# AaltoML/vi-diffusion-processes

Measured on AMD Instinct MI355X. Metric: ELBO steps/sec (T=100k, d=6) at 1/2/4/8 GPU; HBM GB/s vs roofline, higher is better.
Workload: dtype f64; 1 GPU; CVI-DP site-update loop (CVISitesSDE: update_data_sites + update_girsanov_sites + classic_elbo) on double-well SDE trajectories, T=100000, d=6, 64 trajectories per GPU, observation every 50 steps, correlated observation noise (full d x d data sites); trajectories_per_gpu=64, T=100000, d=6, total_trajectories=64

## Files before the change

include/mfgm.h:

```cpp
#ifndef MFGM_H
#define MFGM_H

#include <stddef.h>
#include <stdint.h>

#ifdef __cplusplus
extern "C" {
#endif

typedef struct mfgm_plan mfgm_plan;

#define MFGM_VEC 0
#define MFGM_FULL 1
#define MFGM_SYM 2
#define MFGM_TRI 3

int mfgm_plan_create(int B, int T, int d, int R0, int Rup, mfgm_plan** out);
void mfgm_plan_destroy(mfgm_plan* plan);
int mfgm_plan_describe(const mfgm_plan* plan, int* out6);
size_t mfgm_plan_workspace_bytes(const mfgm_plan* plan);
size_t mfgm_packed_doubles(const mfgm_plan* plan, int kind);

int mfgm_pack(const mfgm_plan* plan, int kind, const double* natural, int n_nodes, double* packed, void* stream);
int mfgm_unpack(const mfgm_plan* plan, int kind, const double* packed, double* natural, int n_nodes, void* stream);
// ... 112 lines not shown
                        double* quad, double* L2, double* y2, void* ws, int* info, void* stream);
int mfgm_cq_factor_pair_stage(const mfgm_plan* plan, int stage, const mfgm_cq_state* q, const mfgm_cq_state* q_next, double* L, double* y,
                              double* L2, double* y2, void* ws, int* info, void* stream);
size_t mfgm_cq_heads_scratch_doubles(const mfgm_plan* plan, int stride);
int mfgm_cq_factor_pair_heads(const mfgm_plan* plan, int stride, const mfgm_cq_state* q, const mfgm_cq_state* q_next, double* L, double* y,
                              double* logdet, double* quad, double* L2, double* y2, double* scratch, size_t scratch_doubles, void* ws, int* info,
                              void* stream);
int mfgm_cq_factor_pair_heads_stage(const mfgm_plan* plan, int stage, int stride, const mfgm_cq_state* q, const mfgm_cq_state* q_next,
                                    double* L, double* y, double* L2, double* y2, double* scratch, size_t scratch_doubles, void* ws, int* info,
                                    void* stream);
int mfgm_cq_selinv_girsanov_alt(const mfgm_plan* plan, int only_level, const mfgm_cq_state* q, const double* L2, const double* y2,
                                const mfgm_sde_params* prm, double* dyn_out, void* ws, void* stream);
int mfgm_cq_selinv_kl(const mfgm_plan* plan, int only_level, const mfgm_cq_state* q, const double* L, const double* y,
                      const mfgm_sde_params* prm, double* Sig, double* x, double* kl_part, double* obs_mu, double* obs_cov, void* ws,
                      void* stream);
int mfgm_mvn_ve_compact(int B, int n_per, int d, const double* mu, const double* cov, const double* y, const double* Sinv, double cst,
                        double* ve, void* stream);

#define MFGM_QUAD_NTHETA 40
typedef struct mfgm_quad_drift {
    int kind, d, nh, pad_;
    double theta[MFGM_QUAD_NTHETA];
    double dt;
    double W[6];
    double logdetQp;
    double mu0[3];
    double P0inv[6];
    double logdetP0;
    double clip_lo, clip_hi;
} mfgm_quad_drift;
// ... 360 lines not shown
```

vi-diffusion-processes_amd/_lib.py:

```python
import ctypes
import os

_HERE = os.path.dirname(os.path.abspath(__file__))
LIB_PATH = os.environ.get("MFGM_LIB") or os.path.join(_HERE, "csrc", "libmfgm.so")

VEC, FULL, SYM, TRI = 0, 1, 2, 3
FACTOR_MATERN12, FACTOR_MATERN32, FACTOR_MATERN52, FACTOR_CONSTANT, FACTOR_HARMONIC = 1, 2, 3, 4, 5
LIK_BERNOULLI, LIK_POISSON, LIK_GAUSSIAN = 1, 2, 3

_lib = None

EXPORTS = {
    "mfgm_version": (ctypes.c_char_p, []),
    "mfgm_plan_create": (ctypes.c_int, [ctypes.c_int] * 5 + [ctypes.POINTER(ctypes.c_void_p)]),
    "mfgm_plan_destroy": (None, [ctypes.c_void_p]),
    "mfgm_plan_describe": (ctypes.c_int, [ctypes.c_void_p, ctypes.POINTER(ctypes.c_int)]),
    "mfgm_plan_workspace_bytes": (ctypes.c_size_t, [ctypes.c_void_p]),
    "mfgm_packed_doubles": (ctypes.c_size_t, [ctypes.c_void_p, ctypes.c_int]),
    "mfgm_pack": (ctypes.c_int, [ctypes.c_void_p, ctypes.c_int, ctypes.c_void_p, ctypes.c_int, ctypes.c_void_p,
                                 ctypes.c_void_p]),
    "mfgm_unpack": (ctypes.c_int, [ctypes.c_void_p, ctypes.c_int, ctypes.c_void_p, ctypes.c_void_p, ctypes.c_int,
                                   ctypes.c_void_p]),
    "mfgm_packed_factor": (ctypes.c_int, [ctypes.c_void_p] * 4 + [ctypes.c_double] * 3 + [ctypes.c_void_p] * 8),
    "mfgm_packed_selinv": (ctypes.c_int, [ctypes.c_void_p] * 9),
# ... 70 lines not shown
    "mfgm_cq_slots": (ctypes.c_int, [ctypes.c_void_p, ctypes.c_void_p, ctypes.c_int, ctypes.c_void_p, ctypes.c_void_p, ctypes.c_void_p]),
    "mfgm_cq_factor": (ctypes.c_int, [ctypes.c_void_p] * 9),
    "mfgm_cq_factor_pipelined": (ctypes.c_int, [ctypes.c_void_p] * 8 + [ctypes.c_int] + [ctypes.c_void_p] * 3),
    "mfgm_quad_linearize": (ctypes.c_int, [ctypes.c_void_p, ctypes.c_int] + [ctypes.c_void_p] * 6),
    "mfgm_quad_kl_scratch_doubles": (ctypes.c_size_t, [ctypes.c_int] * 4),
    "mfgm_quad_kl": (ctypes.c_int, [ctypes.c_void_p, ctypes.c_int, ctypes.c_int] + [ctypes.c_void_p] * 11),
    "mfgm_quad_vdp_lagrange": (ctypes.c_int, [ctypes.c_int] * 3 + [ctypes.c_double] * 2 + [ctypes.c_void_p] * 8),
    "mfgm_quad_esde": (ctypes.c_int, [ctypes.c_void_p, ctypes.c_int] + [ctypes.c_void_p] * 12),
    "mfgm_cq_factor_stage": (ctypes.c_int, [ctypes.c_void_p, ctypes.c_int] + [ctypes.c_void_p] * 6),
    "mfgm_cq_selinv_girsanov": (ctypes.c_int, [ctypes.c_void_p, ctypes.c_int] + [ctypes.c_void_p] * 7),
    "mfgm_cq_factor_pair": (ctypes.c_int, [ctypes.c_void_p] * 12),
    "mfgm_cq_factor_pair_stage": (ctypes.c_int, [ctypes.c_void_p, ctypes.c_int] + [ctypes.c_void_p] * 9),
    "mfgm_cq_heads_scratch_doubles": (ctypes.c_size_t, [ctypes.c_void_p, ctypes.c_int]),
    "mfgm_cq_factor_pair_heads": (ctypes.c_int, [ctypes.c_void_p, ctypes.c_int] + [ctypes.c_void_p] * 9 + [ctypes.c_size_t] + [ctypes.c_void_p] * 3),
    "mfgm_cq_factor_pair_heads_stage": (ctypes.c_int, [ctypes.c_void_p, ctypes.c_int, ctypes.c_int] + [ctypes.c_void_p] * 7 + [ctypes.c_size_t] + [ctypes.c_void_p] * 3),
    "mfgm_cq_selinv_girsanov_alt": (ctypes.c_int, [ctypes.c_void_p, ctypes.c_int] + [ctypes.c_void_p] * 7),
    "mfgm_cq_selinv_kl": (ctypes.c_int, [ctypes.c_void_p, ctypes.c_int] + [ctypes.c_void_p] * 11),
    "mfgm_mvn_ve_compact": (ctypes.c_int, [ctypes.c_int] * 3 + [ctypes.c_void_p] * 4 + [ctypes.c_double, ctypes.c_void_p, ctypes.c_void_p]),
    "mfgm_kf_sites_loglik": (ctypes.c_int, [ctypes.c_void_p] * 15),
    "mfgm_kf_sites_predict": (ctypes.c_int, [ctypes.c_void_p] * 16),
    "mfgm_kf_sites_elbo": (ctypes.c_int, [ctypes.c_void_p] * 9 + [ctypes.c_double] + [ctypes.c_void_p] * 6),
    "mfgm_kf_sites_predict_factored": (ctypes.c_int, [ctypes.c_void_p] * 11),
    "mfgm_sparse_theta": (ctypes.c_int, [ctypes.c_int, ctypes.c_int] + [ctypes.c_void_p] * 9),
    "mfgm_sparse_predict": (ctypes.c_int, [ctypes.c_void_p] * 7),
    "mfgm_cond_predict": (ctypes.c_int, [ctypes.c_int] * 3 + [ctypes.c_void_p] * 11),
    "mfgm_sparse_site_update": (ctypes.c_int, [ctypes.c_void_p] * 3 + [ctypes.c_double] + [ctypes.c_void_p] * 3),
    "mfgm_packed_naturals_to_ssm": (ctypes.c_int, [ctypes.c_void_p] * 11),
    "mfgm_bidiag_scratch_doubles": (ctypes.c_size_t, [ctypes.c_int] * 3),
    "mfgm_bidiag_solve": (ctypes.c_int, [ctypes.c_int] * 3 + [ctypes.c_void_p] * 4 + [ctypes.c_int, ctypes.c_void_p, ctypes.c_void_p]),
    "mfgm_btd_matvec": (ctypes.c_int, [ctypes.c_int] * 3 + [ctypes.c_void_p] * 4 + [ctypes.c_int, ctypes.c_int, ctypes.c_void_p]),
# ... 186 lines not shown
```

vi-diffusion-processes_amd/csrc/mfgm_api_sweeps.hip:

```cpp
#include "mfgm_internal.h"
#include "mfgm_sweeps.h"
#include "mfgm_rows.h"
#include "mfgm_girsanov.h"
#include "mfgm_cq.h"
#include "mfgm_kf.h"

using namespace mfgm;

namespace {

template <int D>
int launch_reduce(const SweepArgs& a, bool has_rhs, bool has_corr, hipStream_t st) {
    dim3 grid(a.lv.Lpad / 64), block(64);
    if (has_rhs) {
        if (has_corr) hipLaunchKernelGGL((k_reduce<D, true, true>), grid, block, 0, st, a);
        else hipLaunchKernelGGL((k_reduce<D, true, false>), grid, block, 0, st, a);
    } else {
        if (has_corr) hipLaunchKernelGGL((k_reduce<D, false, true>), grid, block, 0, st, a);
        else hipLaunchKernelGGL((k_reduce<D, false, false>), grid, block, 0, st, a);
    }
    MFGM_CHECK_LAUNCH();
    return 0;
}

// ... 319 lines not shown
            if (a0.lv.nt >= 2) hipLaunchKernelGGL((k_forward_cq<D, 2>), grid, block, 0, st, a0, q);
            else hipLaunchKernelGGL((k_forward_cq<D>), grid, block, 0, st, a0, q);
        }
        MFGM_CHECK_LAUNCH();
        if (next && !side && !rides) {
            hipLaunchKernelGGL((k_reduce_cq_lean<D>), grid, block, 0, st, an, *next);
            MFGM_CHECK_LAUNCH();
        }
    }
    if (logdet || quad) return sum_level0_partials(P, ws, P.lv[0].Lpad, logdet, quad, st);
    return 0;
}

template <int D>
int cq_factor_pair_impl(const Plan& P, const CqArgs& q, const CqArgs& q2, double* Lg, double* yg, double* logdet, double* quad, double* L2,
                        double* y2, double* ws, int* info, hipStream_t st, int only_stage = -1, double* park = nullptr, int stride = 0) {
    const auto on = [&](int s) { return only_stage < 0 || only_stage == s; };
    const size_t sh = P.off_pair - P.off_Dhat[1];
    double* ws2 = ws + sh;
    SweepArgs a0;
    memset(&a0, 0, sizeof(a0));
    a0.lv = P.lv[0];
    a0.info = info;
    a0.aD = -2.0; a0.aS = -1.0; a0.aR = 1.0;
    a0.Lg = Lg; a0.yg = yg;
    a0.part = (logdet || quad) ? ws + P.off_part[0] : nullptr;
    SweepArgs a1 = a0;
    a1.Lg = L2; a1.yg = y2; a1.part = nullptr;
    bind_up(P, 0, ws, a0);
    bind_up(P, 0, ws2, a1);
    dim3 grid(a0.lv.Lpad / 64), block(64);
    if (on(0) && park) {
        hipLaunchKernelGGL((k_reduce_cq_interior<D>), grid, block, 0, st, a0, q, park, stride);
        MFGM_CHECK_LAUNCH();
        hipLaunchKernelGGL((k_reduce_cq_heads<D>), dim3(grid.x, 2), block, 0, st, a0, q, a1, q2, park, stride);
        MFGM_CHECK_LAUNCH();
    } else if (on(0)) {
        hipLaunchKernelGGL((k_reduce_cq<D>), grid, block, 0, st, a0, q);
        MFGM_CHECK_LAUNCH();
        hipLaunchKernelGGL((k_reduce_cq<D>), grid, block, 0, st, a1, q2);
        MFGM_CHECK_LAUNCH();
    }
    if (on(2))
        if (int rc = coarse_up_pair<D>(P, ws, sh, info, st)) return rc;
    if (!on(1)) {
    } else if constexpr (D <= 6) {
        if (a0.lv.nt >= 1) hipLaunchKernelGGL((k_forward_pair_cq<D, 1>), grid, dim3(128), 0, st, a0, q, a1, q2);
        else hipLaunchKernelGGL((k_forward_pair_cq<D>), grid, dim3(128), 0, st, a0, q, a1, q2);
        MFGM_CHECK_LAUNCH();
    } else {
        if (a0.lv.nt >= 2) {
            hipLaunchKernelGGL((k_forward_cq<D, 2>), grid, block, 0, st, a0, q);
            hipLaunchKernelGGL((k_forward_cq<D, 2>), grid, block, 0, st, a1, q2);
        } else {
            hipLaunchKernelGGL((k_forward_cq<D>), grid, block, 0, st, a0, q);
            hipLaunchKernelGGL((k_forward_cq<D>), grid, block, 0, st, a1, q2);
        }
        MFGM_CHECK_LAUNCH();
    }
    if (logdet || quad)
        if (int rc = sum_level0_partials(P, ws, P.lv[0].Lpad, logdet, quad, st)) return rc;
    if (on(3)) return coarse_down_pair<D>(P, ws, sh, st);
    return 0;
// ... 10 lines not shown
    a.lv = P.lv[0];
    a.Lg = const_cast<double*>(Lg); a.yg = const_cast<double*>(yg); a.aS = -1.0;
    bind_up(P, 0, wsc, a);
    double* fix = ws + P.off_part[0];
    dim3 grid(a.lv.Lpad / 64), block(64);
    if (a.lv.nt >= 2) hipLaunchKernelGGL((k_backward_girsanov_cq<D, 2>), grid, block, 0, st, a, pr, q, fix);
    else hipLaunchKernelGGL((k_backward_girsanov_cq<D>), grid, block, 0, st, a, pr, q, fix);
    MFGM_CHECK_LAUNCH();
    hipLaunchKernelGGL((k_girsanov_fixup_cq<D>), grid, block, 0, st, a.lv, q.dyn_out, (const double*)fix);
    MFGM_CHECK_LAUNCH();
    return 0;
}

template <int D>
int cq_selinv_kl_impl(const Plan& P, const CqArgs& q, const double* Lg, const double* yg, const SdeParams& pr, double* Sig, double* x,
                      double* kl, double* ws, hipStream_t st, int only_level) {
    if (only_level != 0)
        if (int rc = coarse_down<D>(P, ws, true, st)) return rc;
    if (only_level > 0) return 0;
    SweepArgs a;
    memset(&a, 0, sizeof(a));
    a.lv = P.lv[0];
    a.Lg = const_cast<double*>(Lg); a.yg = const_cast<double*>(yg); a.aS = -1.0;
    a.Sigg = Sig; a.mug = x;
    a.part = ws + P.off_part[0];
    bind_up(P, 0, ws, a);
    if (a.lv.nt >= 2) hipLaunchKernelGGL((k_backward_kl_cq<D, 2>), dim3(a.lv.Lpad / 64), dim3(64), 0, st, a, pr, q);
    else hipLaunchKernelGGL((k_backward_kl_cq<D>), dim3(a.lv.Lpad / 64), dim3(64), 0, st, a, pr, q);
    MFGM_CHECK_LAUNCH();
    return sum_level0_partials(P, ws, 0, kl, nullptr, st);
}

template <int D>
int cq_pack_impl(const Plan& P, const double* lin, const double* diag, const double* sub, double* dyn, double* range, hipStream_t st) {
    hipLaunchKernelGGL((k_cq_pack<D>), dim3(P.lv[0].Lpad / 64), dim3(64), 0, st, P.lv[0], lin, diag, sub, dyn, range);
    MFGM_CHECK_LAUNCH();
    return 0;
}
template <int D>
int cq_unpack_impl(const Plan& P, const CqArgs& q, double* lin, double* diag, double* sub, hipStream_t st) {
    hipLaunchKernelGGL((k_cq_unpack<D>), dim3(P.lv[0].Lpad / 64), dim3(64), 0, st, P.lv[0], q, lin, diag, sub);
    MFGM_CHECK_LAUNCH();
    return 0;
// ... 255 lines not shown
                                                  stride)));
}

int mfgm_cq_factor_pair_heads_stage(const mfgm_plan* plan, int stage, int stride, const mfgm_cq_state* q, const mfgm_cq_state* q_next,
                                    double* L, double* y, double* L2, double* y2, double* scratch, size_t scratch_doubles, void* ws, int* info,
                                    void* stream) {
    if (!cq_pair_ok(plan, q, q_next, L, y, L2, y2, ws, info) || !cq_heads_ok(plan, stride, scratch, scratch_doubles) || stage < 0 ||
        stage > 3)
        return 1;
    const Plan& P = plan->p;
    const CqArgs c = cq_args(q), c2 = cq_args(q_next);
    MFGM_DISPATCH_D(P.d, (cq_factor_pair_impl<DD>(P, c, c2, L, y, nullptr, nullptr, L2, y2, (double*)ws, info, (hipStream_t)stream, stage,
                                                  scratch, stride)));
}

int mfgm_cq_selinv_girsanov_alt(const mfgm_plan* plan, int only_level, const mfgm_cq_state* q, const double* L2, const double* y2,
                                const mfgm_sde_params* prm, double* dyn_out, void* ws, void* stream) {
    if (!cq_ok(plan, q) || !L2 || !y2 || !prm || !dyn_out || !ws || dyn_out == q->dyn || prm->kind != 0 || plan->p.off_pair == 0) return 1;
    const Plan& P = plan->p;
    const SdeParams pr = sde_params(prm);
    CqArgs c = cq_args(q);
    c.dyn_out = dyn_out;
    MFGM_DISPATCH_D(P.d, (cq_selinv_girsanov_impl<DD>(P, c, L2, y2, pr, (double*)ws, (hipStream_t)stream, only_level, true)));
}

int mfgm_cq_selinv_kl(const mfgm_plan* plan, int only_level, const mfgm_cq_state* q, const double* L, const double* y,
                      const mfgm_sde_params* prm, double* Sig, double* x, double* kl_part, double* obs_mu, double* obs_cov, void* ws,
                      void* stream) {
    if (!cq_ok(plan, q) || !L || !y || !prm || !kl_part || !ws || prm->kind != 0) return 1;
    if ((obs_mu != nullptr) != (obs_cov != nullptr) || (Sig != nullptr) != (x != nullptr)) return 1;
// ... 261 lines not shown
```

vi-diffusion-processes_amd/csrc/mfgm_cq.h:

```cpp
#pragma once
#include "mfgm_girsanov.h"

namespace mfgm {

struct CqArgs {
    const double* dyn;
    double dOff, sOff;
    const double* p0off;
    const int* slot;
    const double* site_lin;
    const double* site_sym;
    double* dyn_out;
    double* obs_mu;
    double* obs_cov;
    const double* site_lin2;
    const double* site_sym2;
    double* pre_Dhat; double* pre_Rsub; double* pre_S; double* pre_rhat; double* pre_rho;
};

template <int E, int E0, int N>
MFGM_DEV void ld_part(const double* __restrict__ base, int R, int s, LaneRef w, double (&out)[N]) {
    const double* p = base + ((size_t)w.tile * R + s) * (size_t)(E * 64) + (size_t)E0 * 64;
    if (w.nt >= 2) {
#pragma unroll
// ... 524 lines not shown
#pragma unroll
    for (int k = 0; k < MFGM_NTRI(D); ++k) Sig[k] = Pm[k];
    gemm_tn_sym_acc<D>(Ssub, H, -1.0, Sig);
#pragma unroll
    for (int i = 0; i < D; ++i) {
        double t = x[i];
#pragma unroll
        for (int k = 0; k < D; ++k) t = __builtin_fma(-Pm[six(i, k)], tg[k], t);
        x[i] = t;
    }
}

#ifndef MFGM_CQ_SYNC_EVERY
#define MFGM_CQ_SYNC_EVERY 2
#endif
template <int D, bool SYNC>
MFGM_DEV void forward_cq_body(const SweepArgs& a, const CqArgs& q, const int lane, const LaneRef me) {
    constexpr int ET = MFGM_NTRI(D), EF = D * D, E3 = 3 * D;
    const int P = a.lv.P, R = a.lv.R, Lp = a.lv.Lpad, n = a.lv.n;
    const int b = lane / P, p = lane - b * P;
    const int len = min(R, n - p * R);
    const bool sites = (q.slot != nullptr);
    int bad = 0;
    double ssym[ET];
    cq_site_sym<ET>(q, sites, ssym);

    double C[ET], c[D];
#pragma unroll
    for (int e = 0; e < ET; ++e) C[e] = 0.0;
#pragma unroll
    for (int e = 0; e < D; ++e) c[e] = 0.0;
// ... 92 lines not shown
#pragma unroll
            for (int j = 0; j < D; ++j) la.mul(F[tix(j, j)]);
            la.renorm();
#pragma unroll
            for (int j = 0; j < D; ++j) quad = __builtin_fma(h[j], h[j], quad);
            double X[ET], Pm[ET], z[D];
            tri_inverse<D>(F, invd, X);
            tri_t_tri<D>(X, Pm);
#pragma unroll
            for (int i = 0; i < D; ++i) {
                double t = 0.0;
#pragma unroll
                for (int k = i; k < D; ++k) t = __builtin_fma(X[tix(k, i)], h[k], t);
                z[i] = t;
            }
            st_node<ET>(a.Lg, R, s, me, Pm);
            st_node<D>(a.yg, R, s, me, z);
            cq_carry<D>(Pm, z, sdn, has_next ? a.aS : 0.0, q.sOff, C, c);
        }
        if constexpr (SYNC) {
            if ((s & (MFGM_CQ_SYNC_EVERY - 1)) == MFGM_CQ_SYNC_EVERY - 1) __syncthreads();
        }
    }
    if (a.part) {
        a.part[lane] = la.value();
        a.part[Lp + lane] = quad;
    }
    if (bad) flag_not_pd(a.info, a.lv.level, lane);
}
template <int D, int NT = 0>
static __global__ __launch_bounds__(64) void k_forward_cq(SweepArgs a, CqArgs q) {
    const int lane = blockIdx.x * 64 + threadIdx.x;
// ... 166 lines not shown
    const int lane = min((int)blockIdx.x * 64 + l, a.lv.L - 1);
    const LaneRef me{(int)blockIdx.x, lane & 63, NT >= 1 ? 1 : 0};
    if (wave == 0) forward_cq_body<D, true>(a, q, lane, me);
    else reduce_cq_lds_body<D>(a, q, lane, me, lds, l);
}

template <int D, int NT = 0>
static __global__ __launch_bounds__(128) __attribute__((amdgpu_waves_per_eu(2, 2))) void k_forward_pair_cq(SweepArgs a, CqArgs q, SweepArgs a2,
                                                                                                            CqArgs q2) {
    const int wave = threadIdx.x >> 6, l = threadIdx.x & 63;
    const int lane = min((int)blockIdx.x * 64 + l, a.lv.L - 1);
    const LaneRef me{(int)blockIdx.x, lane & 63, NT >= 1 ? 1 : 0};
    if (wave == 0) forward_cq_body<D, true>(a, q, lane, me);
    else forward_cq_body<D, true>(a2, q2, lane, me);
}

template <int D>
MFGM_DEV void backward_s_left_cq(const SweepArgs& a, const CqArgs& q, int R, LaneRef left, const double (&Sn)[MFGM_NTRI(D)],
                                 double (&Gd)[D], double (&SnH)[D * D]) {
    constexpr int ET = MFGM_NTRI(D);
    double H[D * D], Pm[ET], e[D], u[D];
    ld_node<ET>(a.Lg, R, R - 1, left, Pm);
    ld_part<3 * D, 2 * D, D>(q.dyn, R, R - 1, left, Gd);
    const double so = (D == 1) ? 0.0 : q.sOff;
    const double cs = a.aS * so;
#pragma unroll
    for (int i = 0; i < D; ++i) {
        e[i] = a.aS * (Gd[i] - so);
        double t = 0.0;
#pragma unroll
// ... 241 lines not shown
            double Ssub[EF], Sig[ET];
            backward_p_step<D>(Lt, Gd, q.sOff, a.aS, Sn, xn, Sig, Ssub, x);
            if (keep) {
                st_node<D>(a.mug, R, s, me, x);
                st_node<ET>(a.Sigg, R, s, me, Sig);
            }
            if (obs) cq_store_obs<D>(q, sc, x, Sig);
            double v[D], c[D], vn[D];
#pragma unroll
            for (int i = 0; i < D; ++i) { v[i] = Sig[tix(i, i)]; c[i] = Ssub[i * D + i]; vn[i] = Sn[tix(i, i)]; }
            acc += kl_transition<D>(pr, x, v, c, xn, vn);
#pragma unroll
            for (int i = 0; i < D; ++i) xn[i] = x[i];
#pragma unroll
            for (int e = 0; e < ET; ++e) Sn[e] = Sig[e];
        }
    }
    if (p > 0) {
        const LaneRef left = LaneRef::of(lane - 1);
        double Gd[D], Ssub[EF];
        backward_s_left_cq<D>(a, q, R, left, Sn, Gd, Ssub);
        double m[D], v[D], c[D], vn[D];
        up_moments<D>(a, b, p - 1, m, v);
#pragma unroll
        for (int i = 0; i < D; ++i) { c[i] = -Ssub[i * D + i]; vn[i] = Sn[tix(i, i)]; }
        acc += kl_transition<D>(pr, m, v, c, xn, vn);
    } else {
        double tr = 0.0, mh = 0.0;
#pragma unroll
        for (int i = 0; i < D; ++i) {
// ... 129 lines not shown
```

vi-diffusion-processes_amd/packed.py:

```python
import ctypes
import os

import torch

from . import _lib
from ._lib import FULL, SYM, TRI, VEC
from .stamps import wrote


def _ptr(t):
    return ctypes.c_void_p(0 if t is None else t.data_ptr())


def _stream():
    return ctypes.c_void_p(torch.cuda.current_stream().cuda_stream)


def observation_period(time_index):
    ti = torch.as_tensor(time_index)
    if ti.dim() > 1:
        ti = ti.reshape(-1, ti.shape[-1])
        if ti.shape[0] > 1 and not bool((ti == ti[:1]).all()):
            return 0
        ti = ti[0]
# ... 68 lines not shown
        _lib.check(self.lib.mfgm_unpack(self.h, kind, _ptr(packed), _ptr(out), n_nodes, _stream()), "mfgm_unpack")
        return out

    def factor(self, D, S, r=None, aD=1.0, aS=1.0, aR=1.0, want_logdet=True, want_quad=False, out=None, store_G=True,
               moments_only=False):
        out = {} if out is None else out
        form = 1 if (moments_only and self.wide and store_G and os.environ.get("MFGM_INVERSE_FORM", "1") != "0") else 0
        L = out.get("L") if out.get("L") is not None else self.empty(TRI)
        G = None
        if store_G:
            G = out.get("G") if out.get("G") is not None else self.empty(FULL)
        y = None
        if r is not None:
            y = out.get("y") if out.get("y") is not None else self.empty(VEC)
        self.epoch += 1
        logdet = torch.empty(self.B, dtype=torch.float64, device=self.device) if want_logdet else None
        quad = torch.empty(self.B, dtype=torch.float64, device=self.device) if want_quad else None
        _lib.check(self.lib.mfgm_packed_factor_form(self.h, form, _ptr(D), _ptr(S), _ptr(r), float(aD), float(aS), float(aR),
                                                    _ptr(L), _ptr(G), _ptr(y), _ptr(logdet), _ptr(quad), _ptr(self.ws),
                                                    _ptr(self.info), _stream()), "mfgm_packed_factor_form")
        return dict(L=L, G=G, y=y, logdet=logdet, quad=quad, form=form)

    def sparse_factor(self, nat1, nat2, plin, pdiag, psub, want_logdet=True, out=None, packed=False):
        out = {} if out is None else out
        L = out.get("L") if out.get("L") is not None else self.empty(TRI)
        G = out.get("G") if out.get("G") is not None else self.empty(FULL)
        y = out.get("y") if out.get("y") is not None else self.empty(VEC)
        self.epoch += 1
        logdet = torch.empty(self.B, dtype=torch.float64, device=self.device) if want_logdet else None
        if packed:
            _lib.check(self.lib.mfgm_sparse_factor_q(self.h, -1, _ptr(nat1), _ptr(nat2), _ptr(plin), _ptr(pdiag), _ptr(psub), _ptr(L), _ptr(G),
                                                     _ptr(y), _ptr(logdet), None, _ptr(self.ws), _ptr(self.info), _stream()),
                       "mfgm_sparse_factor_q")
        else:
            _lib.check(self.lib.mfgm_sparse_factor(self.h, _ptr(nat1), _ptr(nat2), _ptr(plin), _ptr(pdiag), _ptr(psub), _ptr(L), _ptr(G),
                                                   _ptr(y), _ptr(logdet), None, _ptr(self.ws), _ptr(self.info), _stream()), "mfgm_sparse_factor")
        return dict(L=L, G=G, y=y, logdet=logdet, quad=None, form=1)

    def selinv(self, L, G, y=None, want_sub=True, out=None, form=0):
        out = {} if out is None else out
        Sig = out.get("Sig") if out.get("Sig") is not None else self.empty(SYM)
        Sub = None
        if want_sub:
# ... 253 lines not shown
    def cq_slots(self, node_ids):
        slot = torch.empty(self.lib.mfgm_cq_slot_ints(self.h), dtype=torch.int32, device=self.device)
        dup = torch.zeros(1, dtype=torch.int32, device=self.device)
        _lib.check(self.lib.mfgm_cq_slots(self.h, _ptr(node_ids), node_ids.numel(), _ptr(slot), _ptr(dup), _stream()), "mfgm_cq_slots")
        return None if int(dup.item()) else slot

    def cq_factor(self, cq, want_logdet=True, out=None, use_ahead=False, next_sites=None, side=None):
        out = {} if out is None else out
        L = out.get("L") if out.get("L") is not None else self.empty(TRI)
        y = out.get("y") if out.get("y") is not None else self.empty(VEC)
        self.epoch += 1
        logdet = torch.empty(self.B, dtype=torch.float64, device=self.device) if want_logdet else None
        if not use_ahead and next_sites is None:
            _lib.check(self.lib.mfgm_cq_factor(self.h, ctypes.byref(cq.struct()), _ptr(L), _ptr(y), _ptr(logdet), None, _ptr(self.ws),
                                               _ptr(self.info), _stream()), "mfgm_cq_factor")
            return dict(L=L, y=y, logdet=logdet)
        nxt = None
        if next_sites is not None:
            nxt = cq.struct()
            nxt.site_lin, nxt.site_sym = next_sites[0].data_ptr(), next_sites[1].data_ptr()
        _lib.check(self.lib.mfgm_cq_factor_pipelined(self.h, ctypes.byref(cq.struct()), _ptr(L), _ptr(y), _ptr(logdet), None, _ptr(self.ws),
                                                     _ptr(self.info), 1 if use_ahead else 0, ctypes.byref(nxt) if nxt is not None else None,
                                                     ctypes.c_void_p(side.cuda_stream) if side is not None else None, _stream()),
                   "mfgm_cq_factor_pipelined")
        return dict(L=L, y=y, logdet=logdet)

    def cq_factor_pair(self, cq, next_sites, out=None, out2=None, want_logdet=True, head_stride=None):
        out = {} if out is None else out
        out2 = {} if out2 is None else out2
        L = out.get("L") if out.get("L") is not None else self.empty(TRI)
        y = out.get("y") if out.get("y") is not None else self.empty(VEC)
        L2 = out2.get("L") if out2.get("L") is not None else self.empty(TRI)
        y2 = out2.get("y") if out2.get("y") is not None else self.empty(VEC)
        self.epoch += 1
        logdet = torch.empty(self.B, dtype=torch.float64, device=self.device) if want_logdet else None
        nxt = cq.struct()
        nxt.site_lin, nxt.site_sym = next_sites[0].data_ptr(), next_sites[1].data_ptr()
        if head_stride is not None:
            scratch = self._heads_scratch(int(head_stride))
            _lib.check(self.lib.mfgm_cq_factor_pair_heads(self.h, int(head_stride), ctypes.byref(cq.struct()), ctypes.byref(nxt), _ptr(L), _ptr(y),
                                                          _ptr(logdet), None, _ptr(L2), _ptr(y2), _ptr(scratch), scratch.numel(), _ptr(self.ws),
                                                          _ptr(self.info), _stream()), "mfgm_cq_factor_pair_heads")
            return dict(L=L, y=y, logdet=logdet), dict(L=L2, y=y2)
        _lib.check(self.lib.mfgm_cq_factor_pair(self.h, ctypes.byref(cq.struct()), ctypes.byref(nxt), _ptr(L), _ptr(y), _ptr(logdet), None,
                                                _ptr(L2), _ptr(y2), _ptr(self.ws), _ptr(self.info), _stream()), "mfgm_cq_factor_pair")
        return dict(L=L, y=y, logdet=logdet), dict(L=L2, y=y2)

    def _heads_scratch(self, stride):
        held = getattr(self, "_heads_buf", None)
        if held is None or held[0] != stride:
            n = self.lib.mfgm_cq_heads_scratch_doubles(self.h, stride)
            held = self._heads_buf = (stride, torch.empty(max(int(n), 1), dtype=torch.float64, device=self.device))
        return held[1]

    def cq_selinv_girsanov(self, cq, L, y, prm, dyn_out, only_level=-1, alt=False):
        fn = self.lib.mfgm_cq_selinv_girsanov_alt if alt else self.lib.mfgm_cq_selinv_girsanov
        _lib.check(fn(self.h, int(only_level), ctypes.byref(cq.struct()), _ptr(L), _ptr(y), ctypes.byref(prm),
                      _ptr(dyn_out), _ptr(self.ws), _stream()), "mfgm_cq_selinv_girsanov_alt" if alt else "mfgm_cq_selinv_girsanov")
        return dyn_out

    def cq_selinv_kl(self, cq, L, y, prm, out=None, obs_mu=None, obs_cov=None, only_level=-1, want_marginals=True):
        out = {} if out is None else out
        Sig = x = None
        if want_marginals:
            Sig = out.get("Sig") if out.get("Sig") is not None else self.empty(SYM)
            x = out.get("x") if out.get("x") is not None else self.empty(VEC)
        kl = torch.empty(self.B, dtype=torch.float64, device=self.device)
        _lib.check(self.lib.mfgm_cq_selinv_kl(self.h, int(only_level), ctypes.byref(cq.struct()), _ptr(L), _ptr(y), ctypes.byref(prm), _ptr(Sig),
                                              _ptr(x), _ptr(kl), _ptr(obs_mu), _ptr(obs_cov), _ptr(self.ws), _stream()), "mfgm_cq_selinv_kl")
        return dict(Sig=Sig, x=x, klpart=kl)

    def mvn_ve_compact(self, mu, cov, n_per, y, Sinv, cst, partials=False):
        ve = torch.empty((self.B, (int(n_per) + 255) // 256), dtype=torch.float64, device=self.device)
        _lib.check(self.lib.mfgm_mvn_ve_compact(self.B, int(n_per), self.d, _ptr(mu), _ptr(cov), _ptr(y), _ptr(Sinv), float(cst), _ptr(ve),
                                                _stream()), "mfgm_mvn_ve_compact")
        return ve if partials else ve.sum(-1)

    def cq_elbo(self, ve_part, kl_part, logdet, c):
        out = torch.empty(self.B + 1, dtype=torch.float64, device=self.device)
        _lib.check(self.lib.mfgm_cq_elbo(self.B, int(ve_part.shape[-1]), _ptr(ve_part), _ptr(kl_part), _ptr(logdet), float(c), _ptr(self.info),
                                         _ptr(out), ctypes.c_void_p(out.data_ptr() + 8 * self.B), _stream()), "mfgm_cq_elbo")
        return out[:self.B], out[self.B]

    def site_lerp_to(self, out1, x1, g1, out2, x2, g2, w):
# ... 32 lines not shown
```

vi-diffusion-processes_amd/variational_cvi_sde.py:

```python
import math
import os

import numpy as np
import torch

from . import linalg, quad, tape
from ._lib import FULL, SYM, VEC
from .packed import CqState, Plan, aligned_segment_length, observation_period
from .sde import mvnquad
from .ssm_gaussian_transformations import naturals_to_ssm_params_packed
from .stamps import Stamp, wrote
from .state_space_model import PackedSSM, StateSpaceModel


def grid_indices(time_grid, obs_times):
    tg = torch.as_tensor(time_grid, dtype=torch.float64).cpu()
    ot = torch.as_tensor(obs_times, dtype=torch.float64).cpu()
    idx = torch.searchsorted(tg, ot)
    idx = idx.clamp(max=tg.numel() - 1)
    if not torch.equal(tg[idx], ot):
        raise ValueError("every observation time must be a point of the time grid")
    return idx


# ... 501 lines not shown
        else:
            self._cq.slot, self._cq.site_lin, self._cq.site_sym = keep_sites

    fused_girsanov = os.environ.get("VIDP_FUSED_GIRSANOV", "1") != "0"

    def _sweep_fusion(self):
        pl, prm = self.plan, self._sde_prm
        return self.fused_girsanov and prm is not None and pl.d <= 8 and pl.nlevels >= 2 and prm.kind == 0

    _need_sub = False

    pipelined = os.environ.get("VIDP_PIPELINE", "1") != "0"
    pipe_two_streams = os.environ.get("VIDP_PIPE_STREAMS", "0") == "1"
    pipe_pair = os.environ.get("VIDP_PIPE_PAIR", "1") != "0"
    pair_heads = os.environ.get("VIDP_PAIR_HEADS", "1") != "0"
    pipeline_min_nodes = 200000

    def _pair_head_stride(self):
        q = self._obs_stride
        return q if self.pair_heads and q >= 2 and self.plan.R % q == 0 else None

    def _site_blend(self, cq, lin, sym, lr):
        g1, g2 = self.likelihood.ve_gradients_expectation(self.fx_mus_obs, self.fx_covs_obs, self._obs_flat)
        if self._cq_g2[0] is not g2:
            self._cq_g2 = (g2, self._sym_packed(g2[0]))
        self.plan.site_lerp_to(lin, self._data_nat1, g1.contiguous(), sym, cq.site_sym, self._cq_g2[1], lr)

    def update_data_sites(self, lr: float):
        cq = self._cq_state()
        if cq is None or cq.slot is None:
# ... 48 lines not shown
        pl = self.plan
        obs = cq.slot is not None
        lazy = obs and not want_marginals and os.environ.get("VIDP_LAZY_MARGINALS", "1") != "0"
        if self._q is None:
            ahead = self._ahead
            if (self.pipelined and obs and ahead.lr is not None and self._sde_prm.kind == 0
                    and self.B * self.T >= self.pipeline_min_nodes and self.state_dim <= 6):
                if self.pipe_two_streams and ahead.side is None:
                    ahead.side = torch.cuda.Stream(device=self.device)
                pair = self.pipe_pair and ahead.side is None

                def launch(lin, sym, lr_next):
                    self._site_blend(cq, lin, sym, lr_next)
                    if pair:
                        f, f2 = pl.cq_factor_pair(cq, (lin, sym), out=self._bufs["f"], out2=self._bufs.setdefault("f2", {}),
                                                  head_stride=self._pair_head_stride())
                        self._bufs["f2"].update(L=f2["L"], y=f2["y"])
                        return f, f2
                    return pl.cq_factor(cq, want_logdet=True, out=self._bufs["f"], next_sites=(lin, sym), side=ahead.side)
                f = ahead.make(self._data_nat1, cq, pl, launch, kind=ahead.PAIR if pair else ahead.REDUCE)
                coarse_done = pair
            else:
                f = pl.cq_factor(cq, want_logdet=True, out=self._bufs["f"], use_ahead=ahead.take(self._data_nat1, cq, pl), side=ahead.side)
                coarse_done = False
            self._bufs["f"].update(L=f["L"], y=f["y"])
            s = pl.cq_selinv_kl(cq, f["L"], f["y"], self._sde_prm, out=self._bufs["s"], obs_mu=self.fx_mus_obs if obs else None,
                                obs_cov=self.fx_covs_obs if obs else None, want_marginals=not lazy, only_level=0 if coarse_done else -1)
            if not lazy:
                self._bufs["s"].update(Sig=s["Sig"], x=s["x"])
            self._q = dict(logdetL=f["logdet"], mu=s["x"], Sig=s["Sig"], Sub=None, mom=None, klpart=s["klpart"], epoch=pl.epoch)
            self._obs_fresh = obs
        elif self._q["mu"] is None and not lazy:
            f = self._bufs["f"]
            if self._q.get("epoch") != pl.epoch:
                f = pl.cq_factor(cq, want_logdet=False, out=self._bufs["f"])
                self._q["epoch"] = pl.epoch
            s = pl.cq_selinv_kl(cq, f["L"], f["y"], self._sde_prm, out=self._bufs["s"], obs_mu=self.fx_mus_obs if obs else None,
                                obs_cov=self.fx_covs_obs if obs else None, want_marginals=True)
            self._bufs["s"].update(Sig=s["Sig"], x=s["x"])
            self._q.update(mu=s["x"], Sig=s["Sig"])
        return self._q

    def variational_expectation(self, partials=False):
        cq, lik = self._cq_state(), self.likelihood
        if cq is None or cq.slot is None:
            return super().variational_expectation()
        self._refresh()
        if not self._obs_fresh:
            self._gather_obs()
        return self.plan.mvn_ve_compact(self.fx_mus_obs, self.fx_covs_obs, self.n_obs, self._obs_flat, lik.inv_covariance, lik.ve_constant,
                                        partials=partials)

    def _cq_elbo(self):
# ... 398 lines not shown
```

Measured before the change: 431.3 ELBO steps/s.

## Thin stored Cholesky factors to even nodes and recompute odd ones in backward KL sweep

The paired forward factor kernel now stores the per-node Cholesky factor L and y only at even nodes (plus the last node), which halves the factor writes. The new backward KL kernel rebuilds the odd-node factors on the fly from the stored even node and the dynamics and site data. This trades HBM write and read traffic for redundant Cholesky, triangular-inverse and solve arithmetic in the backward sweep. It is enabled by default for d<=6 on the pipelined pair path, and Python bookkeeping marks a thinned factor so that girsanov selinv refuses to read it.

```diff
diff --git a/include/mfgm.h b/include/mfgm.h
--- a/include/mfgm.h
+++ b/include/mfgm.h
@@ -150,6 +150,12 @@
 int mfgm_cq_selinv_kl(const mfgm_plan* plan, int only_level, const mfgm_cq_state* q, const double* L, const double* y,
                       const mfgm_sde_params* prm, double* Sig, double* x, double* kl_part, double* obs_mu, double* obs_cov, void* ws,
                       void* stream);
+int mfgm_cq_factor_pair_thin(const mfgm_plan* plan, int stage, int stride, const mfgm_cq_state* q, const mfgm_cq_state* q_next, double* L,
+                             double* y, double* logdet, double* quad, double* L2, double* y2, double* scratch, size_t scratch_doubles, void* ws,
+                             int* info, void* stream);
+int mfgm_cq_selinv_kl_thin(const mfgm_plan* plan, int only_level, const mfgm_cq_state* q, const double* L, const double* y,
+                           const mfgm_sde_params* prm, double* Sig, double* x, double* kl_part, double* obs_mu, double* obs_cov, void* ws,
+                           void* stream);
 int mfgm_mvn_ve_compact(int B, int n_per, int d, const double* mu, const double* cov, const double* y, const double* Sinv, double cst,
                         double* ve, void* stream);
 
diff --git a/vi-diffusion-processes_amd/_lib.py b/vi-diffusion-processes_amd/_lib.py
--- a/vi-diffusion-processes_amd/_lib.py
+++ b/vi-diffusion-processes_amd/_lib.py
@@ -108,6 +108,8 @@
     "mfgm_cq_heads_scratch_doubles": (ctypes.c_size_t, [ctypes.c_void_p, ctypes.c_int]),
     "mfgm_cq_factor_pair_heads": (ctypes.c_int, [ctypes.c_void_p, ctypes.c_int] + [ctypes.c_void_p] * 9 + [ctypes.c_size_t] + [ctypes.c_void_p] * 3),
     "mfgm_cq_factor_pair_heads_stage": (ctypes.c_int, [ctypes.c_void_p, ctypes.c_int, ctypes.c_int] + [ctypes.c_void_p] * 7 + [ctypes.c_size_t] + [ctypes.c_void_p] * 3),
+    "mfgm_cq_factor_pair_thin": (ctypes.c_int, [ctypes.c_void_p, ctypes.c_int, ctypes.c_int] + [ctypes.c_void_p] * 9 + [ctypes.c_size_t] + [ctypes.c_void_p] * 3),
+    "mfgm_cq_selinv_kl_thin": (ctypes.c_int, [ctypes.c_void_p, ctypes.c_int] + [ctypes.c_void_p] * 11),
     "mfgm_cq_selinv_girsanov_alt": (ctypes.c_int, [ctypes.c_void_p, ctypes.c_int] + [ctypes.c_void_p] * 7),
     "mfgm_cq_selinv_kl": (ctypes.c_int, [ctypes.c_void_p, ctypes.c_int] + [ctypes.c_void_p] * 11),
     "mfgm_mvn_ve_compact": (ctypes.c_int, [ctypes.c_int] * 3 + [ctypes.c_void_p] * 4 + [ctypes.c_double, ctypes.c_void_p, ctypes.c_void_p]),
diff --git a/vi-diffusion-processes_amd/csrc/mfgm_api_sweeps.hip b/vi-diffusion-processes_amd/csrc/mfgm_api_sweeps.hip
--- a/vi-diffusion-processes_amd/csrc/mfgm_api_sweeps.hip
+++ b/vi-diffusion-processes_amd/csrc/mfgm_api_sweeps.hip
@@ -357,7 +357,8 @@
 
 template <int D>
 int cq_factor_pair_impl(const Plan& P, const CqArgs& q, const CqArgs& q2, double* Lg, double* yg, double* logdet, double* quad, double* L2,
-                        double* y2, double* ws, int* info, hipStream_t st, int only_stage = -1, double* park = nullptr, int stride = 0) {
+                        double* y2, double* ws, int* info, hipStream_t st, int only_stage = -1, double* park = nullptr, int stride = 0,
+                        bool thin = false) {
     const auto on = [&](int s) { return only_stage < 0 || only_stage == s; };
     const size_t sh = P.off_pair - P.off_Dhat[1];
     double* ws2 = ws + sh;
@@ -388,8 +389,13 @@
         if (int rc = coarse_up_pair<D>(P, ws, sh, info, st)) return rc;
     if (!on(1)) {
     } else if constexpr (D <= 6) {
-        if (a0.lv.nt >= 1) hipLaunchKernelGGL((k_forward_pair_cq<D, 1>), grid, dim3(128), 0, st, a0, q, a1, q2);
-        else hipLaunchKernelGGL((k_forward_pair_cq<D>), grid, dim3(128), 0, st, a0, q, a1, q2);
+        const dim3 pair(128);
+        const bool nt1 = a0.lv.nt >= 1;
+        if (thin) {
+            if (nt1) hipLaunchKernelGGL((k_forward_pair_thin_cq<D, 1>), grid, pair, 0, st, a0, q, a1, q2);
+            else hipLaunchKernelGGL((k_forward_pair_thin_cq<D>), grid, pair, 0, st, a0, q, a1, q2);
+        } else if (nt1) hipLaunchKernelGGL((k_forward_pair_cq<D, 1>), grid, pair, 0, st, a0, q, a1, q2);
+        else hipLaunchKernelGGL((k_forward_pair_cq<D>), grid, pair, 0, st, a0, q, a1, q2);
         MFGM_CHECK_LAUNCH();
     } else {
         if (a0.lv.nt >= 2) {
@@ -430,7 +436,8 @@
 
 template <int D>
 int cq_selinv_kl_impl(const Plan& P, const CqArgs& q, const double* Lg, const double* yg, const SdeParams& pr, double* Sig, double* x,
-                      double* kl, double* ws, hipStream_t st, int only_level) {
+                      double* kl, double* ws, hipStream_t st, int only_level, bool thin = false) {
+    if (thin && D > 6) return 1;
     if (only_level != 0)
         if (int rc = coarse_down<D>(P, ws, true, st)) return rc;
     if (only_level > 0) return 0;
@@ -441,8 +448,15 @@
     a.Sigg = Sig; a.mug = x;
     a.part = ws + P.off_part[0];
     bind_up(P, 0, ws, a);
-    if (a.lv.nt >= 2) hipLaunchKernelGGL((k_backward_kl_cq<D, 2>), dim3(a.lv.Lpad / 64), dim3(64), 0, st, a, pr, q);
-    else hipLaunchKernelGGL((k_backward_kl_cq<D>), dim3(a.lv.Lpad / 64), dim3(64), 0, st, a, pr, q);
+    const dim3 grid(a.lv.Lpad / 64), block(64);
+    if (thin) {
+        if constexpr (D <= 6) {
+            a.aD = -2.0; a.aR = 1.0;
+            if (a.lv.nt >= 2) hipLaunchKernelGGL((k_backward_kl_thin_cq<D, 2>), grid, block, 0, st, a, pr, q);
+            else hipLaunchKernelGGL((k_backward_kl_thin_cq<D>), grid, block, 0, st, a, pr, q);
+        }
+    } else if (a.lv.nt >= 2) hipLaunchKernelGGL((k_backward_kl_cq<D, 2>), grid, block, 0, st, a, pr, q);
+    else hipLaunchKernelGGL((k_backward_kl_cq<D>), grid, block, 0, st, a, pr, q);
     MFGM_CHECK_LAUNCH();
     return sum_level0_partials(P, ws, 0, kl, nullptr, st);
 }
@@ -728,6 +742,30 @@
                                                   scratch, stride)));
 }
 
+int mfgm_cq_factor_pair_thin(const mfgm_plan* plan, int stage, int stride, const mfgm_cq_state* q, const mfgm_cq_state* q_next,
+                             double* L, double* y, double* logdet, double* quad, double* L2, double* y2, double* scratch, size_t scratch_doubles,
+                             void* ws, int* info, void* stream) {
+    if (!cq_pair_ok(plan, q, q_next, L, y, L2, y2, ws, info) || plan->p.d > 6 || stage < -1 || stage > 3) return 1;
+    if (stride != 0 && !cq_heads_ok(plan, stride, scratch, scratch_doubles)) return 1;
+    const Plan& P = plan->p;
+    const CqArgs c = cq_args(q), c2 = cq_args(q_next);
+    if (stage >= 0) logdet = quad = nullptr;
+    MFGM_DISPATCH_D(P.d, (cq_factor_pair_impl<DD>(P, c, c2, L, y, logdet, quad, L2, y2, (double*)ws, info, (hipStream_t)stream, stage,
+                                                  stride ? scratch : nullptr, stride, true)));
+}
+
+int mfgm_cq_selinv_kl_thin(const mfgm_plan* plan, int only_level, const mfgm_cq_state* q, const double* L, const double* y,
+                           const mfgm_sde_params* prm, double* Sig, double* x, double* kl_part, double* obs_mu, double* obs_cov, void* ws,
+                           void* stream) {
+    if (!cq_ok(plan, q) || !L || !y || !prm || !kl_part || !ws || prm->kind != 0 || plan->p.d > 6) return 1;
+    if ((obs_mu != nullptr) != (obs_cov != nullptr) || (Sig != nullptr) != (x != nullptr)) return 1;
+    const Plan& P = plan->p;
+    const SdeParams pr = sde_params(prm);
+    CqArgs c = cq_args(q);
+    c.obs_mu = obs_mu; c.obs_cov = obs_cov;
+    MFGM_DISPATCH_D(P.d, (cq_selinv_kl_impl<DD>(P, c, L, y, pr, Sig, x, kl_part, (double*)ws, (hipStream_t)stream, only_level, true)));
+}
+
 int mfgm_cq_selinv_girsanov_alt(const mfgm_plan* plan, int only_level, const mfgm_cq_state* q, const double* L2, const double* y2,
                                 const mfgm_sde_params* prm, double* dyn_out, void* ws, void* stream) {
     if (!cq_ok(plan, q) || !L2 || !y2 || !prm || !dyn_out || !ws || dyn_out == q->dyn || prm->kind != 0 || plan->p.off_pair == 0) return 1;
diff --git a/vi-diffusion-processes_amd/csrc/mfgm_cq.h b/vi-diffusion-processes_amd/csrc/mfgm_cq.h
--- a/vi-diffusion-processes_amd/csrc/mfgm_cq.h
+++ b/vi-diffusion-processes_amd/csrc/mfgm_cq.h
@@ -562,7 +562,8 @@
 #ifndef MFGM_CQ_SYNC_EVERY
 #define MFGM_CQ_SYNC_EVERY 2
 #endif
-template <int D, bool SYNC>
+MFGM_DEV bool cq_kept(int s, int R) { return !(s & 1) || s == R - 1; }
+template <int D, bool SYNC, bool THIN = false>
 MFGM_DEV void forward_cq_body(const SweepArgs& a, const CqArgs& q, const int lane, const LaneRef me) {
     constexpr int ET = MFGM_NTRI(D), EF = D * D, E3 = 3 * D;
     const int P = a.lv.P, R = a.lv.R, Lp = a.lv.Lpad, n = a.lv.n;
@@ -685,8 +686,10 @@
                 for (int k = i; k < D; ++k) t = __builtin_fma(X[tix(k, i)], h[k], t);
                 z[i] = t;
             }
-            st_node<ET>(a.Lg, R, s, me, Pm);
-            st_node<D>(a.yg, R, s, me, z);
+            if (!THIN || cq_kept(s, R)) {
+                st_node<ET>(a.Lg, R, s, me, Pm);
+                st_node<D>(a.yg, R, s, me, z);
+            }
             cq_carry<D>(Pm, z, sdn, has_next ? a.aS : 0.0, q.sOff, C, c);
         }
         if constexpr (SYNC) {
@@ -883,6 +886,15 @@
     if (wave == 0) forward_cq_body<D, true>(a, q, lane, me);
     else forward_cq_body<D, true>(a2, q2, lane, me);
 }
+template <int D, int NT = 0>
+static __global__ __launch_bounds__(128) __attribute__((amdgpu_waves_per_eu(2, 2))) void k_forward_pair_thin_cq(SweepArgs a, CqArgs q, SweepArgs a2,
+                                                                                                                 CqArgs q2) {
+    const int wave = threadIdx.x >> 6, l = threadIdx.x & 63;
+    const int lane = min((int)blockIdx.x * 64 + l, a.lv.L - 1);
+    const LaneRef me{(int)blockIdx.x, lane & 63, NT >= 1 ? 1 : 0};
+    if (wave == 0) forward_cq_body<D, true, true>(a, q, lane, me);
+    else forward_cq_body<D, true>(a2, q2, lane, me);
+}
 
 template <int D>
 MFGM_DEV void backward_s_left_cq(const SweepArgs& a, const CqArgs& q, int R, LaneRef left, const double (&Sn)[MFGM_NTRI(D)],
@@ -1154,6 +1166,157 @@
             for (int i = 0; i < D; ++i) xn[i] = x[i];
 #pragma unroll
             for (int e = 0; e < ET; ++e) Sn[e] = Sig[e];
+        }
+    }
+    if (p > 0) {
+        const LaneRef left = LaneRef::of(lane - 1);
+        double Gd[D], Ssub[EF];
+        backward_s_left_cq<D>(a, q, R, left, Sn, Gd, Ssub);
+        double m[D], v[D], c[D], vn[D];
+        up_moments<D>(a, b, p - 1, m, v);
+#pragma unroll
+        for (int i = 0; i < D; ++i) { c[i] = -Ssub[i * D + i]; vn[i] = Sn[tix(i, i)]; }
+        acc += kl_transition<D>(pr, m, v, c, xn, vn);
+    } else {
+        double tr = 0.0, mh = 0.0;
+#pragma unroll
+        for (int i = 0; i < D; ++i) {
+            double pm = 0.0;
+#pragma unroll
+            for (int j = 0; j < D; ++j) {
+                pm = __builtin_fma(pr.P0inv[six(i, j)], xn[j] - pr.mu0[j], pm);
+                tr = __builtin_fma(pr.P0inv[six(i, j)], Sn[six(i, j)], tr);
+            }
+            mh = __builtin_fma(pm, xn[i] - pr.mu0[i], mh);
+        }
+        acc += 0.5 * (tr + mh + pr.logdetP0);
+    }
+    a.part[lane] = acc;
+}
+
+template <int D>
+MFGM_DEV void cq_forward_step(const double (&Pp)[MFGM_NTRI(D)], const double (&zp)[D], const double (&sdp)[D], const double (&lin)[D],
+                              const double (&dg)[D], double dOff, double sOff, double aD, double aS, double aR, double cnt,
+                              const double (&ssym)[MFGM_NTRI(D)], const double (&sl)[D], double (&Pm)[MFGM_NTRI(D)], double (&z)[D]) {
+    constexpr int ET = MFGM_NTRI(D);
+    double C[ET], c[D], F[ET], h[D], invd[D], X[ET];
+    int bad = 0;
+    cq_carry<D>(Pp, zp, sdp, aS, sOff, C, c);
+#pragma unroll
+    for (int i = 0; i < D; ++i)
+#pragma unroll
+        for (int j = 0; j <= i; ++j) {
+            const double dn = __builtin_fma(cnt, ssym[tix(i, j)], (i == j) ? dg[i] : dOff);
+            F[tix(i, j)] = __builtin_fma(aD, dn, -C[tix(i, j)]);
+        }
+#pragma unroll
+    for (int e = 0; e < D; ++e) h[e] = __builtin_fma(aR, lin[e] + sl[e], -c[e]);
+    chol_inplace<D>(F, invd, bad);
+    trsv_lower<D>(F, invd, h);
+    tri_inverse<D>(F, invd, X);
+    tri_t_tri<D>(X, Pm);
+#pragma unroll
+    for (int i = 0; i < D; ++i) {
+        double t = 0.0;
+#pragma unroll
+        for (int k = i; k < D; ++k) t = __builtin_fma(X[tix(k, i)], h[k], t);
+        z[i] = t;
+    }
+}
+
+template <int D, int NT = 0>
+static __global__ __launch_bounds__(64) void k_backward_kl_thin_cq(SweepArgs a, SdeParams pr, CqArgs q) {
+    constexpr int ET = MFGM_NTRI(D), EF = D * D, E3 = 3 * D;
+    const int lane = blockIdx.x * 64 + threadIdx.x;
+    if (lane >= a.lv.L) return;
+    const LaneRef me{(int)blockIdx.x, (int)threadIdx.x, NT};
+    const int P = a.lv.P, R = a.lv.R, n = a.lv.n;
+    const int b = lane / P, p = lane - b * P;
+    const int len = min(R, n - p * R);
+    const int se = len - 1, top = len - 2;
+    const int uP = a.up.P, uR = a.up.R;
+    const bool sites = (q.slot != nullptr);
+    const bool obs = (sites && q.obs_mu != nullptr);
+    double acc = 0.0;
+    double ssym[ET];
+    cq_site_sym<ET>(q, sites, ssym);
+
+    double Sn[ET], xn[D];
+    {
+        const int ul = b * uP + p / uR, us = p % uR;
+        ld_node<ET, true>(a.uSig, uR, us, LaneRef::of(ul), Sn);
+        ld_node<D, true>(a.umu, uR, us, LaneRef::of(ul), xn);
+    }
+    const bool keep = (a.Sigg != nullptr);
+    if (keep) {
+        st_node<ET>(a.Sigg, R, se, me, Sn);
+        st_node<D>(a.mug, R, se, me, xn);
+    }
+    if (obs) cq_store_obs<D>(q, cq_slot(q.slot, R, se, me), xn, Sn);
+
+    const auto visit = [&](int s, const double (&Pm)[ET], const double (&Gd)[D], double (&x)[D], int sc) {
+        double Ssub[EF], Sig[ET];
+        backward_p_step<D>(Pm, Gd, q.sOff, a.aS, Sn, xn, Sig, Ssub, x);
+        if (keep) {
+            st_node<D>(a.mug, R, s, me, x);
+            st_node<ET>(a.Sigg, R, s, me, Sig);
+        }
+        if (obs) cq_store_obs<D>(q, sc, x, Sig);
+        double v[D], c[D], vn[D];
+#pragma unroll
+        for (int i = 0; i < D; ++i) { v[i] = Sig[tix(i, i)]; c[i] = Ssub[i * D + i]; vn[i] = Sn[tix(i, i)]; }
+        acc += kl_transition<D>(pr, x, v, c, xn, vn);
+#pragma unroll
+        for (int i = 0; i < D; ++i) xn[i] = x[i];
+#pragma unroll
+        for (int e = 0; e < ET; ++e) Sn[e] = Sig[e];
+    };
+
+    double Ln[ET], Gdn[D], yn[D], lo[D], dgo[D], Gdo[D];
+    int sn = -1, so = -1;
+    if (len > 1) {
+        const int e0 = top & ~1;
+        ld_node<ET>(a.Lg, R, e0, me, Ln);
+        ld_part<E3, 2 * D, D>(q.dyn, R, e0, me, Gdn);
+        ld_node<D>(a.yg, R, e0, me, yn);
+        if (obs) sn = cq_slot(q.slot, R, e0, me);
+        if (top & 1) {
+            ld_part<E3, 0, D>(q.dyn, R, top, me, lo);
+            ld_part<E3, D, D>(q.dyn, R, top, me, dgo);
+            ld_part<E3, 2 * D, D>(q.dyn, R, top, me, Gdo);
+            if (sites) so = cq_slot(q.slot, R, top, me);
+        }
+    }
+    for (int e = (R - 2) & ~1; e >= 0; e -= 2) {
+        if (e <= top) {
+            double Lt[ET], z[D], Gd[D];
+#pragma unroll
+            for (int k = 0; k < ET; ++k) Lt[k] = Ln[k];
+#pragma unroll
+            for (int k = 0; k < D; ++k) { Gd[k] = Gdn[k]; z[k] = yn[k]; }
+            const int sc = sn;
+            if (e + 1 <= top) {
+                double Po[ET], x[D], sl[D];
+#pragma unroll
+                for (int i = 0; i < D; ++i) sl[i] = 0.0;
+                if (so >= 0) {
+#pragma unroll
+                    for (int i = 0; i < D; ++i) sl[i] = q.site_lin[(size_t)so * D + i];
+                }
+                cq_forward_step<D>(Lt, z, Gd, lo, dgo, q.dOff, q.sOff, a.aD, a.aS, a.aR, (so >= 0) ? 1.0 : 0.0, ssym, sl, Po, x);
+                visit(e + 1, Po, Gdo, x, so);
+            }
+            if (e > 0) {
+                ld_node<ET>(a.Lg, R, e - 2, me, Ln);
+                ld_part<E3, 2 * D, D>(q.dyn, R, e - 2, me, Gdn);
+                ld_node<D>(a.yg, R, e - 2, me, yn);
+                if (obs) sn = cq_slot(q.slot, R, e - 2, me);
+                ld_part<E3, 0, D>(q.dyn, R, e - 1, me, lo);
+                ld_part<E3, D, D>(q.dyn, R, e - 1, me, dgo);
+                ld_part<E3, 2 * D, D>(q.dyn, R, e - 1, me, Gdo);
+                if (sites) so = cq_slot(q.slot, R, e - 1, me);
+            }
+            visit(e, Lt, Gd, z, sc);
         }
     }
     if (p > 0) {
diff --git a/vi-diffusion-processes_amd/packed.py b/vi-diffusion-processes_amd/packed.py
--- a/vi-diffusion-processes_amd/packed.py
+++ b/vi-diffusion-processes_amd/packed.py
@@ -106,6 +106,7 @@
         if r is not None:
             y = out.get("y") if out.get("y") is not None else self.empty(VEC)
         self.epoch += 1
+        out["thin"] = False
         logdet = torch.empty(self.B, dtype=torch.float64, device=self.device) if want_logdet else None
         quad = torch.empty(self.B, dtype=torch.float64, device=self.device) if want_quad else None
         _lib.check(self.lib.mfgm_packed_factor_form(self.h, form, _ptr(D), _ptr(S), _ptr(r), float(aD), float(aS), float(aR),
@@ -119,6 +120,7 @@
         G = out.get("G") if out.get("G") is not None else self.empty(FULL)
         y = out.get("y") if out.get("y") is not None else self.empty(VEC)
         self.epoch += 1
+        out["thin"] = False
         logdet = torch.empty(self.B, dtype=torch.float64, device=self.device) if want_logdet else None
         if packed:
             _lib.check(self.lib.mfgm_sparse_factor_q(self.h, -1, _ptr(nat1), _ptr(nat2), _ptr(plin), _ptr(pdiag), _ptr(psub), _ptr(L), _ptr(G),
@@ -402,6 +404,7 @@
         if not use_ahead and next_sites is None:
             _lib.check(self.lib.mfgm_cq_factor(self.h, ctypes.byref(cq.struct()), _ptr(L), _ptr(y), _ptr(logdet), None, _ptr(self.ws),
                                                _ptr(self.info), _stream()), "mfgm_cq_factor")
+            out["thin"] = False
             return dict(L=L, y=y, logdet=logdet)
         nxt = None
         if next_sites is not None:
@@ -411,9 +414,10 @@
                                                      _ptr(self.info), 1 if use_ahead else 0, ctypes.byref(nxt) if nxt is not None else None,
                                                      ctypes.c_void_p(side.cuda_stream) if side is not None else None, _stream()),
                    "mfgm_cq_factor_pipelined")
+        out["thin"] = False
         return dict(L=L, y=y, logdet=logdet)
 
-    def cq_factor_pair(self, cq, next_sites, out=None, out2=None, want_logdet=True, head_stride=None):
+    def cq_factor_pair(self, cq, next_sites, out=None, out2=None, want_logdet=True, head_stride=None, thin=False):
         out = {} if out is None else out
         out2 = {} if out2 is None else out2
         L = out.get("L") if out.get("L") is not None else self.empty(TRI)
@@ -424,15 +428,24 @@
         logdet = torch.empty(self.B, dtype=torch.float64, device=self.device) if want_logdet else None
         nxt = cq.struct()
         nxt.site_lin, nxt.site_sym = next_sites[0].data_ptr(), next_sites[1].data_ptr()
-        if head_stride is not None:
-            scratch = self._heads_scratch(int(head_stride))
+        scratch = self._heads_scratch(int(head_stride)) if head_stride is not None else None
+        if thin:
+            _lib.check(self.lib.mfgm_cq_factor_pair_thin(self.h, -1, 0 if head_stride is None else int(head_stride), ctypes.byref(cq.struct()),
+                                                         ctypes.byref(nxt), _ptr(L), _ptr(y), _ptr(logdet), None, _ptr(L2), _ptr(y2), _ptr(scratch),
+                                                         0 if scratch is None else scratch.numel(), _ptr(self.ws), _ptr(self.info), _stream()),
+                       "mfgm_cq_factor_pair_thin")
+        elif head_stride is not None:
             _lib.check(self.lib.mfgm_cq_factor_pair_heads(self.h, int(head_stride), ctypes.byref(cq.struct()), ctypes.byref(nxt), _ptr(L), _ptr(y),
                                                           _ptr(logdet), None, _ptr(L2), _ptr(y2), _ptr(scratch), scratch.numel(), _ptr(self.ws),
                                                           _ptr(self.info), _stream()), "mfgm_cq_factor_pair_heads")
-            return dict(L=L, y=y, logdet=logdet), dict(L=L2, y=y2)
-        _lib.check(self.lib.mfgm_cq_factor_pair(self.h, ctypes.byref(cq.struct()), ctypes.byref(nxt), _ptr(L), _ptr(y), _ptr(logdet), None,
-                                                _ptr(L2), _ptr(y2), _ptr(self.ws), _ptr(self.info), _stream()), "mfgm_cq_factor_pair")
-        return dict(L=L, y=y, logdet=logdet), dict(L=L2, y=y2)
+        else:
+            _lib.check(self.lib.mfgm_cq_factor_pair(self.h, ctypes.byref(cq.struct()), ctypes.byref(nxt), _ptr(L), _ptr(y), _ptr(logdet), None,
+                                                    _ptr(L2), _ptr(y2), _ptr(self.ws), _ptr(self.info), _stream()), "mfgm_cq_factor_pair")
+        out["thin"], out2["thin"] = bool(thin), False
+        first = dict(L=L, y=y, logdet=logdet)
+        if thin:
+            first["thin"] = True
+        return first, dict(L=L2, y=y2)
 
     def _heads_scratch(self, stride):
         held = getattr(self, "_heads_buf", None)
@@ -441,21 +454,24 @@
             held = self._heads_buf = (stride, torch.empty(max(int(n), 1), dtype=torch.float64, device=self.device))
         return held[1]
 
-    def cq_selinv_girsanov(self, cq, L, y, prm, dyn_out, only_level=-1, alt=False):
+    def cq_selinv_girsanov(self, cq, L, y, prm, dyn_out, only_level=-1, alt=False, thin=False):
+        if thin:
+            raise ValueError("cq_selinv_girsanov: a thinned factor is read by cq_selinv_kl alone")
         fn = self.lib.mfgm_cq_selinv_girsanov_alt if alt else self.lib.mfgm_cq_selinv_girsanov
         _lib.check(fn(self.h, int(only_level), ctypes.byref(cq.struct()), _ptr(L), _ptr(y), ctypes.byref(prm),
                       _ptr(dyn_out), _ptr(self.ws), _stream()), "mfgm_cq_selinv_girsanov_alt" if alt else "mfgm_cq_selinv_girsanov")
         return dyn_out
 
-    def cq_selinv_kl(self, cq, L, y, prm, out=None, obs_mu=None, obs_cov=None, only_level=-1, want_marginals=True):
+    def cq_selinv_kl(self, cq, L, y, prm, out=None, obs_mu=None, obs_cov=None, only_level=-1, want_marginals=True, thin=False):
         out = {} if out is None else out
         Sig = x = None
         if want_marginals:
             Sig = out.get("Sig") if out.get("Sig") is not None else self.empty(SYM)
             x = out.get("x") if out.get("x") is not None else self.empty(VEC)
         kl = torch.empty(self.B, dtype=torch.float64, device=self.device)
-        _lib.check(self.lib.mfgm_cq_selinv_kl(self.h, int(only_level), ctypes.byref(cq.struct()), _ptr(L), _ptr(y), ctypes.byref(prm), _ptr(Sig),
-                                              _ptr(x), _ptr(kl), _ptr(obs_mu), _ptr(obs_cov), _ptr(self.ws), _stream()), "mfgm_cq_selinv_kl")
+        fn, name = (self.lib.mfgm_cq_selinv_kl_thin, "mfgm_cq_selinv_kl_thin") if thin else (self.lib.mfgm_cq_selinv_kl, "mfgm_cq_selinv_kl")
+        _lib.check(fn(self.h, int(only_level), ctypes.byref(cq.struct()), _ptr(L), _ptr(y), ctypes.byref(prm), _ptr(Sig),
+                      _ptr(x), _ptr(kl), _ptr(obs_mu), _ptr(obs_cov), _ptr(self.ws), _stream()), name)
         return dict(Sig=Sig, x=x, klpart=kl)
 
     def mvn_ve_compact(self, mu, cov, n_per, y, Sinv, cst, partials=False):
diff --git a/vi-diffusion-processes_amd/variational_cvi_sde.py b/vi-diffusion-processes_amd/variational_cvi_sde.py
--- a/vi-diffusion-processes_amd/variational_cvi_sde.py
+++ b/vi-diffusion-processes_amd/variational_cvi_sde.py
@@ -539,6 +539,7 @@
     pipe_two_streams = os.environ.get("VIDP_PIPE_STREAMS", "0") == "1"
     pipe_pair = os.environ.get("VIDP_PIPE_PAIR", "1") != "0"
     pair_heads = os.environ.get("VIDP_PAIR_HEADS", "1") != "0"
+    thin_factor = os.environ.get("VIDP_THIN_FACTOR", "1") != "0"
     pipeline_min_nodes = 200000
 
     def _pair_head_stride(self):
@@ -617,8 +618,8 @@
                     self._site_blend(cq, lin, sym, lr_next)
                     if pair:
                         f, f2 = pl.cq_factor_pair(cq, (lin, sym), out=self._bufs["f"], out2=self._bufs.setdefault("f2", {}),
-                                                  head_stride=self._pair_head_stride())
-                        self._bufs["f2"].update(L=f2["L"], y=f2["y"])
+                                                  head_stride=self._pair_head_stride(), thin=self.thin_factor and self.state_dim <= 6)
+                        self._bufs["f2"].update(L=f2["L"], y=f2["y"], thin=f2.get("thin", False))
                         return f, f2
                     return pl.cq_factor(cq, want_logdet=True, out=self._bufs["f"], next_sites=(lin, sym), side=ahead.side)
                 f = ahead.make(self._data_nat1, cq, pl, launch, kind=ahead.PAIR if pair else ahead.REDUCE)
@@ -626,9 +627,10 @@
             else:
                 f = pl.cq_factor(cq, want_logdet=True, out=self._bufs["f"], use_ahead=ahead.take(self._data_nat1, cq, pl), side=ahead.side)
                 coarse_done = False
-            self._bufs["f"].update(L=f["L"], y=f["y"])
+            self._bufs["f"].update(L=f["L"], y=f["y"], thin=f.get("thin", False))
             s = pl.cq_selinv_kl(cq, f["L"], f["y"], self._sde_prm, out=self._bufs["s"], obs_mu=self.fx_mus_obs if obs else None,
-                                obs_cov=self.fx_covs_obs if obs else None, want_marginals=not lazy, only_level=0 if coarse_done else -1)
+                                obs_cov=self.fx_covs_obs if obs else None, want_marginals=not lazy, only_level=0 if coarse_done else -1,
+                                thin=f.get("thin", False))
             if not lazy:
                 self._bufs["s"].update(Sig=s["Sig"], x=s["x"])
             self._q = dict(logdetL=f["logdet"], mu=s["x"], Sig=s["Sig"], Sub=None, mom=None, klpart=s["klpart"], epoch=pl.epoch)
@@ -639,7 +641,7 @@
                 f = pl.cq_factor(cq, want_logdet=False, out=self._bufs["f"])
                 self._q["epoch"] = pl.epoch
             s = pl.cq_selinv_kl(cq, f["L"], f["y"], self._sde_prm, out=self._bufs["s"], obs_mu=self.fx_mus_obs if obs else None,
-                                obs_cov=self.fx_covs_obs if obs else None, want_marginals=True)
+                                obs_cov=self.fx_covs_obs if obs else None, want_marginals=True, thin=f.get("thin", False))
             self._bufs["s"].update(Sig=s["Sig"], x=s["x"])
             self._q.update(mu=s["x"], Sig=s["Sig"])
         return self._q
```

After: 467.8 ELBO steps/s, median of 6. 1.08x the previous value.
